# david-mathews-1994/deltarice

Hardware: AMD Instinct MI355X
Metric: encode+decode GB/s (int16 in) (higher is better)
Workload: dtype int16; 1 GPU; 1000000x7000 int16 Gaussian(sigma=10), m=8, 500 chunks of 2000x7000 per GPU, encode then decode, HBM resident; waveforms_per_gpu=1000000, wave_len=7000, rice_m=8, chunks_per_gpu=500, decode_impl=8

## Files before the change

### deltarice_amd/_lib.py

```python
from __future__ import annotations

import ctypes as C
import os

_HERE = os.path.dirname(os.path.abspath(__file__))
LIB_PATH = os.environ.get("DRX_LIB_PATH") or os.path.join(_HERE, "libdeltarice_hip.so")
PLUGIN_PATH = os.path.join(_HERE, "plugin", "libh5deltarice.so")

DRX_OK = 0
STATUS_NAMES = {0: "DRX_OK", 1: "DRX_ERR_ARG", 2: "DRX_ERR_DEVICE", 3: "DRX_ERR_CAPACITY",
                4: "DRX_ERR_CORRUPT", 5: "DRX_ERR_UNSUPPORTED", 6: "DRX_ERR_NOMEM"}
DRX_MAX_TAPS = 64

PATH_LANES_FUSED, PATH_LANES, PATH_BLOCKS, PATH_LONG, PATH_SIMPLE, PATH_IIR, PATH_IIR_FUSED = 1, 2, 4, 8, 16, 32, 64
PATH_SELECT = 128
PATH_GATHER = 256
PATH_STATS = 512
PATH_TRANSCODE = 1024
PATH_WINDOW = 2048
PATH_PULSES = 4096
PATH_WINDOWS = 8192
PATH_BINS = 16384
PATH_STACK = 32768
STACK_COUNT, STACK_SUM, STACK_SUMSQ = range(3)
STACK_COLS = 3
BIN_SUM, BIN_SUMSQ, BIN_MIN, BIN_MAX = range(4)
BIN_COLS = 4
STAT_MIN, STAT_ARGMIN, STAT_MAX, STAT_ARGMAX, STAT_SUM, STAT_SUMSQ, STAT_HEAD_SUM, STAT_HEAD_SUMSQ = range(8)
STAT_COLS = 8
PULSE_START, PULSE_WIDTH, PULSE_PEAK, PULSE_ARGPEAK, PULSE_SUM = range(5)
PULSE_COLS = 5
ENC_TWO_PASS, ENC_SEGMENTS, ENC_FUSED, ENC_PIECES, ENC_STREAM, ENC_STREAM_SEGS = 1, 2, 3, 4, 5, 6
DBG_BINS_LANES = 64
DBG_BINS_ALL_FALLBACK = 128
DBG_NO_LONG_PATHS = 256
DBG_LONG_NOT_BLOCKS = 512
DBG_TRANSCODE_LANES = 1024
DBG_NO_PARALLEL_WALKS = 2048
DBG_NO_PIECES = 4096
DBG_FORCE_SEGMENTS = 8192
DBG_TRANSCODE_ALL_FALLBACK = 16384
DBG_FORCE_PIECES = 32768
DBG_NO_WIDE_FUSED = 65536
DBG_RAGGED_ONE_LANES_LAUNCH = 131072
DBG_STREAM_THREE_WGS = 262144
DBG_FORCE_STREAM = 524288
DBG_REFILTER_SERIAL = 1048576
DBG_IIR_SEPARATE = 2097152
DBG_FORCE_STREAM_SEGS = 4194304
DBG_WALK_BY_SCAN = 8388608
DBG_WALK_BY_CHAINS = 16777216
DBG_GATHER_OTHER_COPY = 33554432
DBG_STATS_LANES = 67108864
DBG_STATS_ALL_FALLBACK = 134217728
DBG_PULSES_LANES = 268435456
DBG_PULSES_ALL_FALLBACK = 536870912
DBG_WINDOWS_LANES = 1073741824
DBG_WINDOWS_ALL_FALLBACK = 2147483648
STATS_FORM_LANES, STATS_FORM_BLOCKS, STATS_FORM_FALLBACK_ALL = 1, 2, 4
PULSES_FORM_LANES, PULSES_FORM_BLOCKS, PULSES_FORM_FALLBACK_ALL = 1, 2, 4
PULSES_STAGE_CAP = 8
WINDOWS_FORM_LANES, WINDOWS_FORM_BLOCKS, WINDOWS_FORM_FALLBACK_ALL = 1, 2, 4
BINS_FORM_LANES, BINS_FORM_BLOCKS, BINS_FORM_FALLBACK_ALL = 1, 2, 4
TRANSCODE_FORM_LANES, TRANSCODE_FORM_BLOCKS, TRANSCODE_FORM_FALLBACK_ALL = 1, 2, 4
TRANSCODE_FORM_REFILTER, TRANSCODE_FORM_REFILTER_SERIAL = 8, 16


class DrxOpts(C.Structure):
    _fields_ = [("rice_k", C.c_uint32), ("wave_len", C.c_int64), ("n_taps", C.c_uint32),
                ("taps", C.c_int32 * DRX_MAX_TAPS)]


class DeltaRiceError(RuntimeError):
    def __init__(self, status: int, msg: str = ""):
        self.status = status
        super().__init__(f"{STATUS_NAMES.get(status, status)}: {msg}")


_vp, _u64, _u32 = C.c_void_p, C.c_uint64, C.c_uint32
SIGNATURES = {
    "drx_version": (C.c_char_p, []),
    "drx_status_str": (C.c_char_p, [C.c_int]),
    "drx_device_count": (C.c_int, []),
    "drx_parse_cd_values": (C.c_int, [C.c_size_t, C.POINTER(C.c_uint), C.POINTER(DrxOpts)]),
    "drx_ctx_create": (C.c_int, [C.c_int, _vp, C.POINTER(_vp)]),
    "drx_ctx_destroy": (None, [_vp]),
    "drx_ctx_synchronize": (C.c_int, [_vp]),
    "drx_ctx_last_error": (C.c_char_p, [_vp]),
    "drx_ctx_stream": (_vp, [_vp]),
    "drx_ctx_device": (C.c_int, [_vp]),
    "drx_ctx_host_staging": (C.c_int, [_vp, C.c_size_t, C.POINTER(_vp)]),
    "drx_ctx_set_option": (C.c_int, [_vp, C.c_char_p, C.c_int64]),
    "drx_plan_create": (C.c_int, [_vp, _u64, C.POINTER(_u32), C.POINTER(_u32), _u32, C.POINTER(_vp)]),
    "drx_plan_create_uniform": (C.c_int, [_vp, _u64, _u32, _u32, _u32, C.POINTER(_vp)]),
    "drx_plan_set_filter": (C.c_int, [_vp, _u32, C.POINTER(C.c_int32)]),
    "drx_plan_destroy": (None, [_vp]),
    "drx_plan_n_chunks": (_u64, [_vp]),
    "drx_plan_total_samples": (_u64, [_vp]),
    "drx_plan_total_waves": (_u64, [_vp]),
    "drx_plan_max_encoded_words": (_u64, [_vp]),
    "drx_plan_wave_words": (_vp, [_vp]),
    "drx_plan_wave_word_off": (_vp, [_vp]),
    "drx_plan_last_decode_path": (C.c_uint32, [_vp]),
    "drx_plan_last_encode_path": (C.c_uint32, [_vp]),
    "drx_plan_last_stats_form": (C.c_uint32, [_vp]),
    "drx_plan_last_pulses_form": (C.c_uint32, [_vp]),
    "drx_plan_last_windows_form": (C.c_uint32, [_vp]),
    "drx_plan_last_windows_listed": (C.c_uint32, [_vp]),
    "drx_plan_last_bins_form": (C.c_uint32, [_vp]),
    "drx_plan_last_bins_listed": (C.c_uint32, [_vp]),
    "drx_plan_last_transcode_form": (C.c_uint32, [_vp]),
    "drx_plan_last_transcode_listed": (C.c_uint32, [_vp]),
    "drx_plan_last_pulses_listed": (C.c_uint32, [_vp]),
    "drx_plan_last_pulses_redone": (C.c_uint32, [_vp]),
    "drx_plan_read_wave_words": (C.c_int, [_vp, C.POINTER(_u32)]),
# ... 51 lines not shown
```

### deltarice_amd/csrc/drx_decode_kernels.hip

```cpp
#include <hip/hip_runtime.h>
#include <stdint.h>

#include <algorithm>
#include <type_traits>

#include "drx_internal.h"
#include "drx_device.h"
#include "drx_lane_stream.h"
#include "drx_walk.h"

namespace drx {

__global__ __launch_bounds__(64) void k_decode_simple(Geom G, const uint32_t *__restrict__ in,
                                                      const uint64_t *__restrict__ wave_off,
                                                      const uint32_t *__restrict__ wave_words, DevStatus *st,
                                                      int16_t *__restrict__ out, const uint32_t *__restrict__ only) {
    const uint64_t g = (uint64_t)blockIdx.x * 64u + threadIdx.x;
    if (g >= G.total_waves) return;
    if (only && !only[g]) return;
    const WaveRef r = locate(G, g);
    const uint32_t *s = in + wave_off[g] + 1;
    const uint32_t n = wave_words[g];
    int16_t *y = out + r.sample_off;
    int16_t hist[64];
// ... 512 lines not shown
    set_limits();
    auto commit_if_fits = [&]() __attribute__((always_inline)) {
        const uint32_t avail = (flw - ((~Q) >> 5)) & WMASK;
        if (pneed && avail <= (uint32_t)(RW - LW)) {
            store_piece(pv);
            pneed = false;
        }
    };
    auto group_refill = [&]() __attribute__((always_inline)) {
        if (__any((int32_t)(Q - Q_need) <= 0)) {
            commit_if_fits();
            wave_sync();
            sync_refill();
            set_limits();
        }
    };
    for (; t0 + T <= hi_min && t0 < steps; t0 += T) {
#pragma unroll 1
        for (int tg = 0; tg < T; tg += GS) {
            group_refill();
            decode_group(std::false_type{}, std::false_type{}, tg, 0u);
        }
        Q_end = (t0 + (uint32_t)T == hi_step) ? Q : Q_end;
        wave_sync();
        commit_if_fits();
        wave_sync();
        set_limits();
        if (!pneed) {
            const bool last = !(t0 + 2u * T <= hi_min && t0 + T < steps);
            const uint32_t avail = (flw - ((~Q) >> 5)) & WMASK;
            pneed = (flw < endw) && (!last || avail <= (uint32_t)(RW - LW));
            if (pneed) load_piece(pv);
        }
#pragma unroll
        for (int i = 0; i < PPS; ++i) {
            const int st = i * SPI + lane / PPS, p = lane % PPS;
            const uint4 v = orow16(st, p);
            store16(outg + wo_off[i] + t0, v);
        }
        wave_sync();
    }
    commit_if_fits();
    pneed = false;
    wave_sync();
    for (; t0 < steps; t0 += T) edge_round(t0);
    if (active && len && (((0u - Q_end) - 32u * s0 + 31u) >> 5) != n) atomicOr(&st->err, kErrCorrupt);
}

std::vector<uint2> decode_plan_ragged(Geom &G, const ChunkDesc *d) {
    const uint64_t n = G.n_chunks;
    uint32_t max_groups = 0, max_len = 0;
    for (uint64_t c = 0; c < n; ++c) {
        max_groups = std::max(max_groups, (d[c].n_waves + 63u) / 64u);
        max_len = std::max(max_len, d[c].wave_len);
    }
    G.max_groups = max_groups;
    G.max_wave_len64 = 64ull * max_len;
    std::vector<uint32_t> by_len(n);
    for (uint64_t c = 0; c < n; ++c) by_len[c] = (uint32_t)c;
    std::stable_sort(by_len.begin(), by_len.end(), [&](uint32_t a, uint32_t b) { return d[a].wave_len > d[b].wave_len; });
    std::vector<uint2> order;
    uint64_t n_long_groups = 0;
    for (uint32_t c : by_len)
        for (uint32_t j = 0; j < (d[c].n_waves + 63u) / 64u; ++j) {
            order.push_back(make_uint2(c, j));
            if (d[c].wave_len > kWalkShortLen) ++n_long_groups;
        }
    if (order.size() <= 0x7fffffffull) {
        G.rag_groups = (uint32_t)order.size();
        G.rag_groups_long = (uint32_t)n_long_groups;
    } else {
        order.clear();
    }
    return order;
}

enum class Dec { Simple, Blocks, Long, LanesFused, Lanes, LanesSplit };
enum class Walk { None, InLaunch, Parallel, Serial };
struct DecodeRoute {
    Dec dec;
    Walk walk;
    WalkRoute par;
    bool gen;
};

static DecodeRoute route_decode(const Geom &G, int impl, bool tables_ready, bool have_pw, bool have_blk, bool have_side) {
    DecodeRoute R{};
    R.gen = G.n_taps != 0;
    R.par = route_walk(G, tables_ready, have_pw);
    const bool simple = impl == 0 || (R.gen && !G.fast_taps);
    const bool want_fused = !tables_ready && impl == 8;
    const bool blocks = !simple && !(G.dbg & (DRX_DBG_NO_LONG_PATHS | DRX_DBG_LONG_NOT_BLOCKS)) && have_blk && blocks_batch(G) && (!R.gen || (G.iir_tab && G.iir_state));
    const bool longp = !simple && !blocks && !R.gen && !(G.dbg & DRX_DBG_NO_LONG_PATHS) && G.uniform && long_waveform_batch(G.total_waves, G.u_wave_len);
    const bool sparse = !G.uniform && (uint64_t)G.n_chunks * G.max_groups > 8ull * ((G.total_waves + 63u) / 64u) + 4096ull;
    R.dec = simple ? Dec::Simple : (blocks ? Dec::Blocks : (longp ? Dec::Long : Dec::Lanes));
    const bool parallel = R.par.chunk_wide || R.par.blocks;
    if (R.dec == Dec::Lanes && want_fused && !sparse && !parallel) R.dec = Dec::LanesFused;
    R.walk = tables_ready ? Walk::None : (R.dec == Dec::LanesFused ? Walk::InLaunch : (parallel ? Walk::Parallel : Walk::Serial));
    if (R.dec == Dec::Lanes && R.par.chunk_wide && R.par.blocks && have_side && G.rag_order && G.rag_groups_long &&
        G.rag_groups_long < G.rag_groups && !(G.dbg & DRX_DBG_RAGGED_ONE_LANES_LAUNCH)) R.dec = Dec::LanesSplit;
    return R;
}

hipError_t launch_decode(const StreamCall &c, int16_t *d_out, uint64_t *d_granules, int impl, void *d_blk, const SideStream *side,
                         uint32_t *path_out) {
    const Geom &G = *c.G;
    const hipStream_t s = c.s;
    uint32_t path_dummy = 0;
    uint32_t &path = path_out ? *path_out : path_dummy;
    path = 0;
    if (G.total_waves == 0) return hipSuccess;
    mark(c.ev, 0, s);
    const DecodeRoute R = route_decode(G, impl, c.tables_ready, c.d_pw != nullptr, d_blk != nullptr, side && side->s);
    const bool gen = R.gen;
    const unsigned nb_plain = blocks_for(G.total_waves, 64);

    auto launch_lanes = [&](const StreamCall &v, unsigned nb) {
        path |= DRX_PATH_LANES;
        if (gen)
            k_decode_lanes<false, true><<<nb, 64, 0, v.s>>>(*v.G, v.d_in, v.in_words, v.d_chunk_word_off, v.d_wave_off, v.d_wave_words, nullptr, nullptr, v.d_status, d_out);
        else
            k_decode_lanes<false><<<nb, 64, 0, v.s>>>(*v.G, v.d_in, v.in_words, v.d_chunk_word_off, v.d_wave_off, v.d_wave_words, nullptr, nullptr, v.d_status, d_out);
    };

    if (R.walk == Walk::InLaunch) {
        hipError_t e = hipMemsetAsync(d_granules, 0, (G.total_waves + 2) * sizeof(uint64_t), s);
        if (e != hipSuccess) return e;
    } else if (R.walk == Walk::Parallel) {
        const bool split = R.dec == Dec::LanesSplit;
        hipError_t e = walk_scratch_reset(G, c.d_pw, s);
        if (e != hipSuccess) return e;
        const bool forked = R.par.chunk_wide && R.par.blocks && side && side->s;
        hipStream_t spw = forked ? side->s : s;
        if (forked) {
            if ((e = hipEventRecord(side->fork, s)) != hipSuccess) return e;
            if ((e = hipStreamWaitEvent(side->s, side->fork, 0)) != hipSuccess) return e;
        }
        if (R.par.chunk_wide) launch_walk_chunk_wide(c.on(spw), R.par.by_chains);
        if (split) {
            Geom Gl = G;
            Gl.rag_groups = G.rag_groups_long;
            launch_lanes(c.view(Gl).on(spw), Gl.rag_groups);
        }
        if (forked && (e = hipEventRecord(side->join, side->s)) != hipSuccess) {
            (void)hipStreamSynchronize(side->s);
            return e;
        }
        if (R.par.blocks) launch_walk_blocks(c);
        if (split) {
            mark(c.ev, 1, s);
            Geom Gs = G;
            Gs.rag_order = G.rag_order + G.rag_groups_long;
            Gs.rag_groups = G.rag_groups - G.rag_groups_long;
            launch_lanes(c.view(Gs), Gs.rag_groups);
        }
        if (forked && (e = hipStreamWaitEvent(s, side->join, 0)) != hipSuccess) {
            (void)hipStreamSynchronize(side->s);
            return e;
        }
    } else if (R.walk == Walk::Serial) {
        launch_walk_serial(c);
    }
    if (R.dec != Dec::LanesSplit) mark(c.ev, 1, s);

    switch (R.dec) {
    case Dec::LanesFused: {
        uint32_t *ticket = reinterpret_cast<uint32_t *>(d_granules + G.total_waves);
        unsigned n_walk, groups;
        unsigned nb;
        if (G.uniform) {
            n_walk = (G.u_wave_len <= kWalkShortLen) ? (unsigned)G.n_chunks : blocks_for(G.n_chunks, kWalkChains);
            groups = (G.u_n_waves + 63u) / 64u;
            const uint32_t full = G.u_n_waves >> 6, rem = G.u_n_waves & 63u;
            nb = n_walk + (unsigned)(G.n_chunks * full) + (rem ? (unsigned)((G.n_chunks + 64u / rem - 1u) / (64u / rem)) : 0u);
        } else {
            n_walk = G.n_short + blocks_for(G.n_long, kWalkChains);
            groups = G.max_groups;
            nb = n_walk + (unsigned)(G.n_chunks * groups);
        }
        path |= DRX_PATH_LANES_FUSED;
        if (gen)
            k_decode_lanes<true, true><<<nb, 64, 0, s>>>(G, c.d_in, c.in_words, c.d_chunk_word_off, c.d_wave_off, c.d_wave_words, d_granules, ticket, c.d_status, d_out);
        else
            k_decode_lanes<true><<<nb, 64, 0, s>>>(G, c.d_in, c.in_words, c.d_chunk_word_off, c.d_wave_off, c.d_wave_words, d_granules, ticket, c.d_status, d_out);
        break;
    }
    case Dec::Blocks: {
        const uint32_t *fail = nullptr, *suspect = nullptr;
        bool fused = false;
        hipError_t e = launch_decode_blocks(c, d_blk, d_out, &fail, &suspect, gen, &fused);
        if (e != hipSuccess) return e;
        path |= DRX_PATH_BLOCKS | (gen ? (fused ? DRX_PATH_IIR_FUSED : DRX_PATH_IIR) : 0u);
        k_decode_long<<<(unsigned)G.total_waves, kLongThreads, 0, s>>>(G, c.d_in, c.d_wave_off, c.d_wave_words, c.d_status, d_out, fail, suspect, gen ? 1u : 0u);
        if (gen) {
            if (!fused && (e = launch_iir(G, G.iir_chunk_tile_base, G.iir_n_tiles, G.iir_tab, G.iir_state, fail, c.d_status, d_out, s)) != hipSuccess) return e;
            k_decode_simple<<<nb_plain, 64, 0, s>>>(G, c.d_in, c.d_wave_off, c.d_wave_words, c.d_status, d_out, fail);
        }
        break;
    }
    case Dec::Long:
        path |= DRX_PATH_LONG;
        k_decode_long<<<(unsigned)G.total_waves, kLongThreads, 0, s>>>(G, c.d_in, c.d_wave_off, c.d_wave_words, c.d_status, d_out, nullptr, nullptr, 0u);
// ... 18 lines not shown
```

### deltarice_amd/csrc/drx_internal.h

```cpp
#ifndef DRX_INTERNAL_H
#define DRX_INTERNAL_H

#include <hip/hip_runtime.h>
#include <stdint.h>

#include <type_traits>
#include <vector>

#include "../../include/deltarice_hip.h"

namespace drx {

struct ChunkDesc {
    uint64_t sample_off;
    uint64_t wave_base;
    uint32_t n_samples;
    uint32_t wave_len;
    uint32_t n_waves;
    uint32_t pad_;
};

struct Geom {
    const ChunkDesc *chunks;
    uint64_t n_chunks;
// ... 191 lines not shown
                              int64_t thr, bool neg, uint32_t min_width, uint32_t max_pulses, uint32_t *d_count, int64_t *d_out,
                              uint32_t *form_out);
uint64_t pulses_blocks_scratch_bytes(const Geom &G);
uint64_t pulses_blocks_staging_bytes(const Geom &G, uint32_t max_pulses);
hipError_t launch_pulses_blocks(const StreamCall &c, void *d_blk, void *d_ptab, void *d_pstage, const int64_t *d_thr, uint64_t thr_stride,
                                int64_t thr, bool neg, uint32_t min_width, uint32_t max_pulses, uint32_t *d_count, int64_t *d_out,
                                BlkFallbackList *list_out);
hipError_t launch_estimate_words(const Geom &G, const int16_t *d_in, unsigned long long *d_words16, hipStream_t s);
hipError_t launch_chunk_offsets(const Geom &G, const uint32_t *d_wave_words, uint32_t *d_wave_rel, uint64_t *d_chunk_words,
                                uint64_t *d_chunk_word_off, uint64_t out_cap, DevStatus *d_status, hipStream_t s);
struct TrcScratch {
    uint64_t *chunk_words;
    unsigned long long *est;
    uint32_t *words, *rel;
    uint64_t bytes;
};
inline TrcScratch trc_scratch_view(const Geom &G, void *base) {
    const uint64_t W = G.total_waves ? G.total_waves : 1, C = G.n_chunks + 1;
    TrcScratch t;
    t.chunk_words = (uint64_t *)base;
    t.est = (unsigned long long *)(t.chunk_words + C);
    t.words = (uint32_t *)(t.est + 16);
    t.rel = t.words + W;
    t.bytes = (C + 16) * sizeof(uint64_t) + 2 * W * sizeof(uint32_t);
    return t;
}
hipError_t launch_transcode(const StreamCall &c, uint32_t k2, const TrcScratch &t, const EncOut &out, void *d_blk, void *d_tb, uint32_t *form_out);
hipError_t launch_estimate_words_encoded(const StreamCall &c, unsigned long long *d_est, void *d_blk, void *d_tb, uint32_t *form_out);
uint64_t trc_blocks_scratch_bytes(const Geom &G);
hipError_t launch_trc_blocks_sizes(const StreamCall &c, void *d_blk, void *d_tb, uint32_t k2, const TrcScratch &t, uint32_t *d_out_wave_words,
                                   unsigned long long *d_est, BlkFallbackList *list_out);
hipError_t launch_trc_blocks_pack(const StreamCall &c, void *d_blk, void *d_tb, uint32_t k2, const TrcScratch &t, const EncOut &out);
struct RefilterTarget {
    uint32_t n_taps;
    const int32_t *taps;
};
hipError_t launch_refilter(const StreamCall &c, uint32_t k2, const RefilterTarget &T, const TrcScratch &t, const EncOut &out, uint32_t *form_out);
hipError_t launch_estimate_words_refiltered(const StreamCall &c, const RefilterTarget &T, unsigned long long *d_est, uint32_t *form_out);

hipError_t launch_encode_fused(const EncodeCall &c, int wide, uint64_t *d_scan);

constexpr uint32_t kEsRingWords = 2496;
constexpr uint64_t kEsMinUnits = 8192;
hipError_t launch_encode_stream(const EncodeCall &c, uint64_t *d_scan);

constexpr uint32_t kEsSegWaves = 4;
constexpr uint32_t kEsSegMinLen = 1024, kEsSegMaxLen = 7168;
struct EsSegShape { uint32_t seg_len, nseg, tpw; };
__host__ __device__ inline EsSegShape es_seg_shape(uint32_t L, uint32_t seg_target) {
    EsSegShape sh;
    uint32_t n = (L + seg_target - 1u) / seg_target;
    n = n ? n : 1u;
    const uint32_t dn = n / kEsSegWaves * kEsSegWaves, up = (n + kEsSegWaves - 1u) / kEsSegWaves * kEsSegWaves;
    n = up;
    if (dn && dn != up) {
        const uint64_t sd = (L + dn - 1u) / dn, su = (L + up - 1u) / up;
        const uint64_t pen_dn = sd > seg_target ? (sd - seg_target) * 55u : 0u, pen_up = su < seg_target ? (seg_target - su) * 40u : 0u;
        if (sd * 57u <= (uint64_t)seg_target * 67u && pen_dn < pen_up) n = dn;
    }
    sh.seg_len = (((L + n - 1u) / n) + 7u) & ~7u;
    sh.nseg = (L + sh.seg_len - 1u) / sh.seg_len;
    sh.tpw = (sh.nseg + kEsSegWaves - 1u) / kEsSegWaves;
    return sh;
}
inline bool stream_segs_admits(const Geom &G) { return G.uniform && (G.n_taps == 0 || G.enc_fast) && G.u_wave_len >= 64u &&
                                                       G.total_waves * es_seg_shape(G.u_wave_len, kEsSegMinLen).tpw < 0xffff0000ull; }
constexpr uint32_t kEsSegsFromLen = 20480;
inline uint64_t segs_scan_words(const Geom &G, uint32_t seg_target) { return 3 * G.total_waves * es_seg_shape(G.u_wave_len, seg_target).tpw + 192; }
hipError_t launch_encode_stream_segs(const EncodeCall &c, uint32_t seg_target, uint64_t *d_scan);

bool long_batch_admits(const Geom &G);
bool long_batch(const Geom &G);
uint64_t long_batch_units(const Geom &G);
std::vector<uint64_t> segments_plan_ragged(Geom &G, const ChunkDesc *host_chunks);
hipError_t launch_encode_long(const EncodeCall &c, uint32_t *d_wave_rel, uint64_t *d_chunk_words, uint32_t *d_seg_bits,
                              uint64_t *d_seg_pos);

struct SideStream {
    hipStream_t s;
    hipEvent_t fork, join;
};
hipError_t launch_decode(const StreamCall &c, int16_t *d_out, uint64_t *d_granules, int impl, void *d_blk, const SideStream *side,
                         uint32_t *path_out = nullptr);
bool blocks_batch(const Geom &G, double lane_us = 0.06, bool any_filter = false);
std::vector<uint32_t> blocks_plan_ragged(Geom &G, const ChunkDesc *host_chunks);
uint64_t blocks_scratch_bytes(const Geom &G);
uint64_t blocks_total_slots(const Geom &G);
hipError_t launch_decode_blocks(const StreamCall &c, void *d_blk, int16_t *d_out, const uint32_t **fail_out,
                                const uint32_t **suspect_out, bool resid, bool *fused_out);
constexpr uint32_t kBlkMaxClasses = 32;
struct BlkTables {
    uint32_t *fail, *suspect, *ends;
    uint64_t *state;
};
struct BlkClassLaunch {
    uint32_t *info;
    const uint32_t *list;
    uint32_t n_waves;
    int nt, sw;
    uint32_t spw, run_len;
    unsigned grid;
};
template <class F> inline void blk_dispatch(int nt, int sw, F f) {
    auto by_sw = [&](auto nt_tag) {
        switch (sw) {
            case 9: f(nt_tag, std::integral_constant<int, 9>{}); break;
            case 11: f(nt_tag, std::integral_constant<int, 11>{}); break;
            case 15: f(nt_tag, std::integral_constant<int, 15>{}); break;
            default: f(nt_tag, std::integral_constant<int, 19>{}); break;
        }
    };
    if (nt == 64) by_sw(std::integral_constant<int, 64>{});
    else if (nt == 128) by_sw(std::integral_constant<int, 128>{});
    else by_sw(std::integral_constant<int, 256>{});
}
hipError_t blocks_prepare(const Geom &G, uint64_t in_words, const uint32_t *d_wave_words, void *d_blk, hipStream_t s, BlkTables *T,
                          BlkClassLaunch *launches, uint32_t *n_launches);
uint32_t blocks_iir_tab_words();
void blocks_iir_tables(const uint32_t fast_nt[3], uint32_t t0neg, uint32_t *tab);
constexpr uint32_t kPcWaves = 8;
constexpr uint32_t kPcRunSamples = 7168;
constexpr uint32_t kPcMaxRun = 16;
constexpr uint32_t kPcSegSamples = 8192;
constexpr uint32_t kPcWholeLen = 10240;
constexpr uint32_t kPcMinLen = 64;
__host__ __device__ inline uint32_t pc_seg_samples(uint32_t k) {
    if (k <= 3u) return kPcSegSamples;
    const uint32_t s = (131072u / (2u * k + 9u)) & ~511u;
    return s < 512u ? 512u : s;
}
__host__ __device__ inline uint32_t pc_run_samples(uint32_t k) { return k <= 3u ? kPcRunSamples : pc_seg_samples(k) - 512u; }
__host__ __device__ inline uint32_t pc_whole_len(uint32_t k) { return k <= 3u ? kPcWholeLen : 65536u / (k + 4u); }
__host__ __device__ inline uint32_t pc_max_len(uint32_t k) { return pc_seg_samples(k) * kPcWaves; }
struct PieceShape {
    uint32_t run;
    uint32_t segs;
    uint32_t parts;
    uint32_t seg_len;
    uint32_t pieces;
    uint32_t wgs;
};
__host__ __device__ inline bool piece_packable(uint32_t L) { return L >= 8u && L < 512u && (L & 7u) == 0u; }
__host__ __device__ inline PieceShape piece_shape(uint32_t L, uint32_t W, uint32_t k, bool packed) {
    PieceShape s;
    s.parts = 1u;
    const uint32_t run_samples = pc_run_samples(k), seg_samples = pc_seg_samples(k), max_len = pc_max_len(k);
    if (packed) {
        const uint32_t bits = k <= 3u ? 9u : k + 6u;
        uint32_t by_samples = run_samples / L, by_words = 2000u / (1u + (bits * L + 31u) / 32u);
        by_samples = by_samples ? by_samples : 1u;
        by_words = by_words ? by_words : 1u;
        s.run = by_samples < by_words ? by_samples : by_words;
        s.segs = 1u;
        s.seg_len = L;
        s.pieces = (W + s.run - 1u) / s.run;
        s.wgs = (s.pieces + kPcWaves - 1u) / kPcWaves;
    } else if (L <= run_samples / 2u) {
        s.run = run_samples / L < kPcMaxRun ? run_samples / L : kPcMaxRun;
        s.segs = 1u;
        s.seg_len = L;
        s.pieces = (W + s.run - 1u) / s.run;
        s.wgs = (s.pieces + kPcWaves - 1u) / kPcWaves;
    } else if (L <= max_len) {
        const uint32_t need = L <= pc_whole_len(k) ? 1u : (L + seg_samples - 1u) / seg_samples;
        s.run = 1u;
        s.segs = 1u;
// ... 40 lines not shown
```

### include/deltarice_hip.h

```cpp
#ifndef DELTARICE_HIP_H
#define DELTARICE_HIP_H

#include <stddef.h>
#include <stdint.h>

#ifdef __cplusplus
extern "C" {
#endif

#define DRX_FILTER_ID 32025
#define DRX_MAX_TAPS 64

typedef struct drx_ctx drx_ctx;
typedef struct drx_plan drx_plan;

typedef enum {
    DRX_OK = 0,
    DRX_ERR_ARG = 1,
    DRX_ERR_DEVICE = 2,
    DRX_ERR_CAPACITY = 3,
    DRX_ERR_CORRUPT = 4,
    DRX_ERR_UNSUPPORTED = 5,
    DRX_ERR_NOMEM = 6
} drx_status;
// ... 131 lines not shown
#define DRX_PULSE_PEAK 2
#define DRX_PULSE_ARGPEAK 3
#define DRX_PULSE_SUM 4
#define DRX_PULSE_COLS 5
drx_status drx_find_pulses(drx_plan *plan, const uint32_t *d_in, uint64_t in_words, const uint64_t *d_chunk_word_off,
                           const int64_t *d_thr, uint64_t thr_stride, int64_t thr, int32_t polarity, uint32_t min_width,
                           uint32_t max_pulses, uint32_t *d_count, int64_t *d_out);
#define DRX_PULSES_FORM_LANES 1u
#define DRX_PULSES_FORM_BLOCKS 2u
#define DRX_PULSES_FORM_FALLBACK_ALL 4u
uint32_t drx_plan_last_pulses_form(const drx_plan *plan);
#define DRX_PULSES_STAGE_CAP 8u
uint32_t drx_plan_last_pulses_listed(const drx_plan *plan);
uint32_t drx_plan_last_pulses_redone(const drx_plan *plan);
drx_status drx_find_pulses_with_wave_words(drx_plan *plan, const uint32_t *d_in, uint64_t in_words,
                                           const uint64_t *d_chunk_word_off, const uint32_t *d_wave_words, const int64_t *d_thr,
                                           uint64_t thr_stride, int64_t thr, int32_t polarity, uint32_t min_width,
                                           uint32_t max_pulses, uint32_t *d_count, int64_t *d_out);

drx_status drx_transcode(drx_plan *plan, const uint32_t *d_in, uint64_t in_words, const uint64_t *d_chunk_word_off,
                         uint32_t new_rice_k, uint32_t *d_out, uint64_t out_cap_words, uint64_t *d_out_chunk_word_off,
                         uint32_t *d_out_wave_words);
drx_status drx_transcode_with_wave_words(drx_plan *plan, const uint32_t *d_in, uint64_t in_words, const uint64_t *d_chunk_word_off,
                                         const uint32_t *d_wave_words, uint32_t new_rice_k, uint32_t *d_out, uint64_t out_cap_words,
                                         uint64_t *d_out_chunk_word_off, uint32_t *d_out_wave_words);
drx_status drx_transcode_filter(drx_plan *plan, const uint32_t *d_in, uint64_t in_words, const uint64_t *d_chunk_word_off,
                                uint32_t new_rice_k, uint32_t new_n_taps, const int32_t *new_taps, uint32_t *d_out,
                                uint64_t out_cap_words, uint64_t *d_out_chunk_word_off, uint32_t *d_out_wave_words);
drx_status drx_transcode_filter_with_wave_words(drx_plan *plan, const uint32_t *d_in, uint64_t in_words,
                                                const uint64_t *d_chunk_word_off, const uint32_t *d_wave_words, uint32_t new_rice_k,
                                                uint32_t new_n_taps, const int32_t *new_taps, uint32_t *d_out, uint64_t out_cap_words,
                                                uint64_t *d_out_chunk_word_off, uint32_t *d_out_wave_words);
#define DRX_TRANSCODE_FORM_LANES 1u
#define DRX_TRANSCODE_FORM_BLOCKS 2u
#define DRX_TRANSCODE_FORM_FALLBACK_ALL 4u
#define DRX_TRANSCODE_FORM_REFILTER 8u
#define DRX_TRANSCODE_FORM_REFILTER_SERIAL 16u
uint32_t drx_plan_last_transcode_form(const drx_plan *plan);
uint32_t drx_plan_last_transcode_listed(const drx_plan *plan);
drx_status drx_estimate_words_encoded(drx_plan *plan, const uint32_t *d_in, uint64_t in_words, const uint64_t *d_chunk_word_off,
                                      const uint32_t *d_wave_words, uint64_t words_out[16]);
drx_status drx_estimate_words_encoded_filter(drx_plan *plan, const uint32_t *d_in, uint64_t in_words, const uint64_t *d_chunk_word_off,
                                             const uint32_t *d_wave_words, uint32_t new_n_taps, const int32_t *new_taps,
                                             uint64_t words_out[16]);

drx_status drx_estimate_words(drx_plan *plan, const int16_t *d_in, uint64_t words_out[16]);

drx_status drx_plan_finish(drx_plan *plan, uint64_t *total_words);

const uint32_t *drx_plan_wave_words(const drx_plan *plan);
const uint64_t *drx_plan_wave_word_off(const drx_plan *plan);
#define DRX_PATH_LANES_FUSED 1u
#define DRX_PATH_LANES 2u
#define DRX_PATH_BLOCKS 4u
#define DRX_PATH_LONG 8u
#define DRX_PATH_SIMPLE 16u
#define DRX_PATH_IIR 32u
#define DRX_PATH_IIR_FUSED 64u
#define DRX_PATH_SELECT 128u
#define DRX_PATH_GATHER 256u
#define DRX_PATH_STATS 512u
#define DRX_PATH_TRANSCODE 1024u
#define DRX_PATH_WINDOW 2048u
#define DRX_PATH_PULSES 4096u
#define DRX_PATH_WINDOWS 8192u
#define DRX_PATH_BINS 16384u
#define DRX_PATH_STACK 32768u
uint32_t drx_plan_last_decode_path(const drx_plan *plan);
#define DRX_ENC_TWO_PASS 1u
#define DRX_ENC_SEGMENTS 2u
#define DRX_ENC_FUSED 3u
#define DRX_ENC_PIECES 4u
#define DRX_ENC_STREAM 5u
#define DRX_ENC_STREAM_SEGS 6u
uint32_t drx_plan_last_encode_path(const drx_plan *plan);
drx_status drx_plan_read_wave_words(drx_plan *plan, uint32_t *host_out);

drx_status drx_filter_chunk_host(drx_ctx *ctx, int reverse, size_t cd_nelmts,
                                 const unsigned *cd_values, const void *in, size_t nbytes,
                                 void **out, size_t *out_bytes);

drx_status drx_plan_last_timings(drx_plan *plan, float ms[4]);

#define DRX_DBG_BINS_LANES 64u
#define DRX_DBG_BINS_ALL_FALLBACK 128u
#define DRX_DBG_NO_LONG_PATHS 256u
#define DRX_DBG_LONG_NOT_BLOCKS 512u
#define DRX_DBG_TRANSCODE_LANES 1024u
#define DRX_DBG_NO_PARALLEL_WALKS 2048u
#define DRX_DBG_NO_PIECES 4096u
#define DRX_DBG_FORCE_SEGMENTS 8192u
#define DRX_DBG_TRANSCODE_ALL_FALLBACK 16384u
#define DRX_DBG_FORCE_PIECES 32768u
#define DRX_DBG_NO_WIDE_FUSED 65536u
#define DRX_DBG_RAGGED_ONE_LANES_LAUNCH 131072u
#define DRX_DBG_STREAM_THREE_WGS 262144u
#define DRX_DBG_FORCE_STREAM 524288u
#define DRX_DBG_REFILTER_SERIAL 1048576u
#define DRX_DBG_IIR_SEPARATE 2097152u
#define DRX_DBG_FORCE_STREAM_SEGS 4194304u
#define DRX_DBG_WALK_BY_SCAN 8388608u
#define DRX_DBG_WALK_BY_CHAINS 16777216u
#define DRX_DBG_GATHER_OTHER_COPY 33554432u
#define DRX_DBG_STATS_LANES 67108864u
#define DRX_DBG_STATS_ALL_FALLBACK 134217728u
#define DRX_DBG_PULSES_LANES 268435456u
#define DRX_DBG_PULSES_ALL_FALLBACK 536870912u
#define DRX_DBG_WINDOWS_LANES 1073741824u
#define DRX_DBG_WINDOWS_ALL_FALLBACK 2147483648u
drx_status drx_ctx_set_option(drx_ctx *ctx, const char *key, int64_t value);

#ifdef __cplusplus
}
#endif
#endif
```

Baseline: 1557 GB/s.

## Add lane-per-wave decode kernel with smaller LDS footprint for eight waves per CU

Adds a new lanes decode kernel that shrinks the per-wavefront shared-memory ring and output staging so eight wavefronts fit per CU, decodes two Rice symbols per step in the steady state, and prefetches the next input piece into registers while the current round's output is written. It is routed in when the lanes path is chosen with impl 8 and the total work is deep enough relative to the longest wave, with debug flags to force or disable it. The kernel is considerably more complex, with edge rounds handled separately, and a smaller ring means more frequent refills.

```diff
diff --git a/deltarice_amd/_lib.py b/deltarice_amd/_lib.py
--- a/deltarice_amd/_lib.py
+++ b/deltarice_amd/_lib.py
@@ -31,6 +31,8 @@
 PULSE_START, PULSE_WIDTH, PULSE_PEAK, PULSE_ARGPEAK, PULSE_SUM = range(5)
 PULSE_COLS = 5
 ENC_TWO_PASS, ENC_SEGMENTS, ENC_FUSED, ENC_PIECES, ENC_STREAM, ENC_STREAM_SEGS = 1, 2, 3, 4, 5, 6
+DBG_LANES_EIGHT_PER_CU = 16
+DBG_LANES_SIX_PER_CU = 32
 DBG_BINS_LANES = 64
 DBG_BINS_ALL_FALLBACK = 128
 DBG_NO_LONG_PATHS = 256
diff --git a/deltarice_amd/csrc/drx_decode_kernels.hip b/deltarice_amd/csrc/drx_decode_kernels.hip
--- a/deltarice_amd/csrc/drx_decode_kernels.hip
+++ b/deltarice_amd/csrc/drx_decode_kernels.hip
@@ -618,6 +618,7 @@
     Walk walk;
     WalkRoute par;
     bool gen;
+    bool lanes8;
 };
 
 static DecodeRoute route_decode(const Geom &G, int impl, bool tables_ready, bool have_pw, bool have_blk, bool have_side) {
@@ -635,6 +636,11 @@
     R.walk = tables_ready ? Walk::None : (R.dec == Dec::LanesFused ? Walk::InLaunch : (parallel ? Walk::Parallel : Walk::Serial));
     if (R.dec == Dec::Lanes && R.par.chunk_wide && R.par.blocks && have_side && G.rag_order && G.rag_groups_long &&
         G.rag_groups_long < G.rag_groups && !(G.dbg & DRX_DBG_RAGGED_ONE_LANES_LAUNCH)) R.dec = Dec::LanesSplit;
+    constexpr uint64_t kLaneSlots = 98304;
+    const uint64_t longest = G.uniform ? G.u_wave_len : G.max_wave_len64 / 64u;
+    const bool deep = longest * kLaneSlots <= G.total_samples;
+    R.lanes8 = (R.dec == Dec::Lanes || R.dec == Dec::LanesSplit) && !R.gen && impl == 8 && !(G.dbg & DRX_DBG_LANES_SIX_PER_CU) &&
+               (deep || (G.dbg & DRX_DBG_LANES_EIGHT_PER_CU));
     return R;
 }
 
@@ -653,7 +659,9 @@
 
     auto launch_lanes = [&](const StreamCall &v, unsigned nb) {
         path |= DRX_PATH_LANES;
-        if (gen)
+        if (R.lanes8)
+            launch_decode_lanes8(v, nb, d_out);
+        else if (gen)
             k_decode_lanes<false, true><<<nb, 64, 0, v.s>>>(*v.G, v.d_in, v.in_words, v.d_chunk_word_off, v.d_wave_off, v.d_wave_words, nullptr, nullptr, v.d_status, d_out);
         else
             k_decode_lanes<false><<<nb, 64, 0, v.s>>>(*v.G, v.d_in, v.in_words, v.d_chunk_word_off, v.d_wave_off, v.d_wave_words, nullptr, nullptr, v.d_status, d_out);
diff --git a/deltarice_amd/csrc/drx_decode_lanes8.hip b/deltarice_amd/csrc/drx_decode_lanes8.hip
--- /dev/null
+++ b/deltarice_amd/csrc/drx_decode_lanes8.hip
@@ -0,0 +1,316 @@
+#include <hip/hip_runtime.h>
+#include <stdint.h>
+
+#include <type_traits>
+
+#include "drx_internal.h"
+#include "drx_device.h"
+
+namespace drx {
+
+__global__ __launch_bounds__(64, 1) void k_decode_lanes8(Geom G, const uint32_t *__restrict__ in, uint64_t in_words,
+                                                         const uint64_t *__restrict__ wave_off,
+                                                         const uint32_t *__restrict__ wave_words, DevStatus *st,
+                                                         int16_t *__restrict__ out) {
+    constexpr int RW = 64;
+    constexpr int LW = 32;
+    constexpr int T = 64;
+    constexpr int GS = 16;
+    constexpr int LOG_RW = 6;
+    constexpr int OSW = GS / 2 + 4;
+    constexpr int PPS = T / 8;
+    constexpr int SPI = 64 / PPS;
+    constexpr int NV = LW / 4;
+    constexpr uint32_t WMASK = (1u << 27) - 1u;
+    constexpr uint32_t NEED_AT = GS + 2;
+    static_assert(T % GS == 0 && RW - LW >= GS + 2, "round length / ring slack");
+    static_assert(GS == 16 && PPS == 8, "a group is two 16-byte pieces of every row");
+    __shared__ uint32_t ring_all[(RW + 2) * 64];
+    uint32_t *const ring = ring_all + 64;
+    __shared__ __attribute__((aligned(16))) uint32_t obuf[64 * OSW];
+    uint64_t *tab_off = reinterpret_cast<uint64_t *>(obuf);
+    uint32_t *tab_lo = obuf + 128, *tab_hi = obuf + 192;
+    static_assert(64 * OSW >= 256, "tables fit in obuf");
+    static_assert(sizeof(ring_all) + sizeof(obuf) <= 20480, "eight wavefronts per CU");
+
+    const int lane = lane_id();
+    const uint32_t k = G.k;
+    typedef uint32_t u32x4v __attribute__((ext_vector_type(4)));
+    typedef u32x4v __attribute__((address_space(1))) g_uint4;
+    typedef int16_t __attribute__((address_space(1))) g_i16;
+    g_i16 *const outg = (g_i16 *)out;
+    uint64_t g;
+    bool active;
+    uint32_t len = 0, n = 0;
+    uint64_t S = 1, ooff = 0;
+    const uint32_t wave_idx = blockIdx.x;
+    if (!G.uniform && G.rag_order) {
+        if (wave_idx >= G.rag_groups) return;
+        const uint2 e = G.rag_order[wave_idx];
+        const ChunkDesc d = G.chunks[e.x];
+        const uint32_t idx = e.y * 64u + (uint32_t)lane;
+        active = idx < d.n_waves;
+        g = d.wave_base + idx;
+        if (active) {
+            len = (idx + 1 == d.n_waves) ? (d.n_samples - idx * d.wave_len) : d.wave_len;
+            ooff = d.sample_off + (uint64_t)idx * d.wave_len;
+            S = wave_off[g] + 1u;
+            n = wave_words[g];
+        }
+    } else {
+        g = (uint64_t)wave_idx * 64u + lane;
+        active = g < G.total_waves;
+        if (active) {
+            const WaveRef r = locate(G, g);
+            len = r.len;
+            ooff = r.sample_off;
+            S = wave_off[g] + 1u;
+            n = wave_words[g];
+        }
+    }
+    const uint32_t phi = active ? (uint32_t)((((uintptr_t)out >> 1) + ooff) & (uint64_t)(T - 1)) : 0u;
+    const uint32_t steps = wave_max_u32(len + phi);
+    const uint32_t lo_max = wave_max_u32(phi);
+    const uint32_t hi_min = ~wave_max_u32(~(phi + len));
+    uint64_t wo_off[PPS];
+    uint32_t wo_lo[PPS], wo_hi[PPS];
+    tab_off[lane] = ooff - phi;
+    tab_lo[lane] = phi;
+    tab_hi[lane] = phi + len;
+    wave_sync();
+#pragma unroll
+    for (int i = 0; i < PPS; ++i) {
+        const int st_i = i * SPI + lane / PPS, p = lane % PPS;
+        wo_off[i] = tab_off[st_i] + 8u * (uint32_t)p;
+        wo_lo[i] = tab_lo[st_i];
+        wo_hi[i] = tab_hi[st_i];
+    }
+    wave_sync();
+
+    const uint64_t A = (S & ~(uint64_t)(RW - 1)) - (uint64_t)RW;
+    const uint32_t s0 = (uint32_t)(S - A);
+    const uint32_t endw = s0 + n;
+    uint32_t flw = s0 & ~(uint32_t)(LW - 1);
+    const bool in_vec_ok = ((uintptr_t)in & 15u) == 0;
+    uint32_t *myring = ring + lane;
+    typedef uint16_t __attribute__((may_alias)) u16a;
+    u16a *myout = reinterpret_cast<u16a *>(obuf + lane * OSW);
+
+    uint4 v[PPS] = {};
+    const int my_group = (lane % PPS) >> 1;
+    const uint32_t *my_rows = obuf + (lane / PPS) * OSW + 4 * (lane & 1);
+    auto read_back = [&](int tg) __attribute__((always_inline)) {
+        if (tg / GS == my_group) {
+#pragma unroll
+            for (int i = 0; i < PPS; ++i) v[i] = *reinterpret_cast<const uint4 *>(my_rows + i * SPI * OSW);
+        }
+    };
+
+    auto load_piece = [&](uint4 (&pv)[NV]) {
+        const uint64_t a = A + flw;
+        if (in_vec_ok && a + (uint32_t)LW <= in_words) {
+#pragma unroll
+            for (int j = 0; j < NV; ++j) pv[j] = *reinterpret_cast<const uint4 *>(in + a + 4 * j);
+        } else {
+#pragma unroll
+            for (int j = 0; j < NV; ++j) {
+                pv[j].x = (a + 4 * j + 0 < in_words) ? in[a + 4 * j + 0] : 0u;
+                pv[j].y = (a + 4 * j + 1 < in_words) ? in[a + 4 * j + 1] : 0u;
+                pv[j].z = (a + 4 * j + 2 < in_words) ? in[a + 4 * j + 2] : 0u;
+                pv[j].w = (a + 4 * j + 3 < in_words) ? in[a + 4 * j + 3] : 0u;
+            }
+        }
+    };
+    auto store_piece = [&](const uint4 (&pv)[NV]) {
+        const uint32_t r0 = (uint32_t)RW - (flw & (uint32_t)(RW - 1));
+        uint32_t *dst = myring + r0 * 64u;
+#pragma unroll
+        for (int j = 0; j < NV; ++j) {
+            dst[-(4 * j + 0) * 64] = pv[j].x; dst[-(4 * j + 1) * 64] = pv[j].y;
+            dst[-(4 * j + 2) * 64] = pv[j].z; dst[-(4 * j + 3) * 64] = pv[j].w;
+        }
+        if (r0 == (uint32_t)RW) {
+            myring[0] = pv[0].x;
+            myring[-64] = pv[0].y;
+        }
+        flw += (uint32_t)LW;
+    };
+
+    uint32_t Q = 0u - 32u * s0;
+    uint32_t Q_need;
+    auto set_limits = [&]() __attribute__((always_inline)) {
+        const bool more = flw < endw;
+        Q_need = more ? ~(32u * (flw - NEED_AT + 1u)) : Q - 0x7fffffffu;
+    };
+    auto sync_refill = [&]() __attribute__((always_inline)) {
+        for (;;) {
+            const uint32_t avail = (flw - ((~Q) >> 5)) & WMASK;
+            const bool more = flw < endw;
+            if (!__any(more && avail < NEED_AT)) break;
+            if (more && avail <= (uint32_t)(RW - LW)) {
+                uint4 pv[NV];
+                load_piece(pv);
+                store_piece(pv);
+            }
+            wave_sync();
+        }
+    };
+
+    {
+        uint4 pv[NV];
+        for (int i = 0; i < RW / LW; ++i) {
+            if (__ballot(flw < endw && flw + (uint32_t)LW <= s0 + (uint32_t)RW) == 0) break;
+            if (flw < endw && flw + (uint32_t)LW <= s0 + (uint32_t)RW) {
+                load_piece(pv);
+                store_piece(pv);
+            }
+        }
+        wave_sync();
+    }
+    int32_t acc = 0;
+
+    const uint32_t hi_step = phi + len;
+    uint32_t Q_end = 0;
+    auto decode_group = [&](auto first_tag, auto edge_tag, int tg, uint32_t tcur) __attribute__((always_inline)) {
+        constexpr bool FIRST = decltype(first_tag)::value;
+        constexpr bool EDGE = decltype(edge_tag)::value;
+        if (!FIRST) {
+#pragma unroll
+            for (int u = 0; u < GS; u += 2) {
+                const uint32_t row = __builtin_amdgcn_ubfe(Q, 5u, (uint32_t)LOG_RW);
+                const uint32_t *wp = myring + row * 64u;
+                const uint32_t lo = wp[0], hi = wp[64], lo2 = wp[-64];
+                const uint32_t winA = __builtin_amdgcn_alignbit(hi, lo, Q);
+                const uint32_t winB = __builtin_amdgcn_alignbit(lo, lo2, Q);
+                const uint32_t q1 = ffbh(winA);
+                const uint32_t kk1 = (winA < (1u << 24)) ? 16u : k;
+                const uint32_t nu1 = ~(q1 + kk1);
+                const uint32_t win2 = __builtin_amdgcn_alignbit(winA, winB, nu1);
+                const uint32_t q2 = ffbh(win2);
+                const uint32_t kk2 = (win2 < (1u << 24)) ? 16u : k;
+                const uint32_t nu2 = ~(q2 + kk2);
+                if constexpr (EDGE) {
+                    Q_end = (tcur + (uint32_t)u + 1u == hi_step) ? Q + nu1 : Q_end;
+                    Q_end = (tcur + (uint32_t)u + 2u == hi_step) ? Q + nu1 + nu2 : Q_end;
+                }
+                asm("v_add3_u32 %0, %1, %2, %3" : "=v"(Q) : "v"(Q), "v"(nu1), "v"(nu2));
+                const uint32_t z1 = (q1 << kk1) + __builtin_amdgcn_ubfe(winA, nu1, kk1);
+                const uint32_t z2 = (q2 << kk2) + __builtin_amdgcn_ubfe(win2, nu2, kk2);
+                acc += (int32_t)(z1 >> 1) ^ -(int32_t)(z1 & 1u);
+                const uint32_t a1 = (uint32_t)acc;
+                acc += (int32_t)(z2 >> 1) ^ -(int32_t)(z2 & 1u);
+                *reinterpret_cast<uint32_t *>(myout + u) = __builtin_amdgcn_perm((uint32_t)acc, a1, 0x05040100u);
+            }
+            return;
+        }
+#pragma unroll
+        for (int u = 0; u < GS; ++u) {
+            const uint32_t row = __builtin_amdgcn_ubfe(Q, 5u, (uint32_t)LOG_RW);
+            const uint32_t *wp = myring + row * 64u;
+            const uint32_t lo = wp[0], hi = wp[64];
+            const uint32_t win = __builtin_amdgcn_alignbit(hi, lo, Q);
+            const uint32_t q = ffbh(win);
+            const bool esc = win < (1u << 24);
+            const uint32_t kk = esc ? 16u : k;
+            const uint32_t used = q + kk + 1u;
+            const uint32_t rem = __builtin_amdgcn_ubfe(win, 32u - used, kk);
+            const uint32_t z = (q << kk) + rem;
+            const int32_t d = (int32_t)(z >> 1) ^ -(int32_t)(z & 1u);
+            const bool act = (uint32_t)(tg + u) >= phi;
+            acc = act ? acc + d : acc;
+            Q = act ? Q - used : Q;
+            if constexpr (EDGE) Q_end = (tcur + (uint32_t)u + 1u == hi_step) ? Q : Q_end;
+            myout[u] = (uint16_t)acc;
+        }
+    };
+
+    auto emit_masked = [&](g_i16 *dst, uint32_t lo, uint32_t hi, uint32_t t0, const uint4 &x) __attribute__((always_inline)) {
+        const int p = lane % PPS;
+        const uint32_t tpos = t0 + 8u * (uint32_t)p;
+        if (tpos + 8u > lo && tpos < hi) {
+            if (tpos >= lo && tpos + 8u <= hi) {
+                *(g_uint4 *)dst = (u32x4v){x.x, x.y, x.z, x.w};
+            } else {
+                const uint32_t w[4] = {x.x, x.y, x.z, x.w};
+#pragma unroll
+                for (int j = 0; j < 8; ++j)
+                    if (tpos + (uint32_t)j >= lo && tpos + (uint32_t)j < hi)
+                        dst[j] = (int16_t)(w[j >> 1] >> (16 * (j & 1)));
+            }
+        }
+    };
+    auto edge_round = [&](auto first_tag, uint32_t t0) __attribute__((always_inline)) {
+#pragma unroll 1
+        for (int tg = 0; tg < T; tg += GS) {
+            sync_refill();
+            decode_group(first_tag, std::true_type{}, tg, t0 + (uint32_t)tg);
+            wave_sync();
+            read_back(tg);
+            wave_sync();
+        }
+        if (t0 >= lo_max && t0 + T <= hi_min) {
+#pragma unroll
+            for (int i = 0; i < PPS; ++i) *(g_uint4 *)(outg + wo_off[i] + t0) = (u32x4v){v[i].x, v[i].y, v[i].z, v[i].w};
+        } else {
+#pragma unroll
+            for (int i = 0; i < PPS; ++i) emit_masked(outg + wo_off[i] + t0, wo_lo[i], wo_hi[i], t0, v[i]);
+        }
+    };
+
+    if (steps > 0) edge_round(std::true_type{}, 0u);
+    uint32_t t0 = T;
+    for (; t0 < steps && !(t0 >= lo_max && t0 + T <= hi_min); t0 += T) edge_round(std::false_type{}, t0);
+
+    uint4 pv[NV];
+    bool pneed = false;
+    set_limits();
+    auto commit_if_fits = [&]() __attribute__((always_inline)) {
+        const uint32_t avail = (flw - ((~Q) >> 5)) & WMASK;
+        if (pneed && avail <= (uint32_t)(RW - LW)) {
+            store_piece(pv);
+            pneed = false;
+        }
+    };
+    auto group_refill = [&]() __attribute__((always_inline)) {
+        if (__any((int32_t)(Q - Q_need) <= 0)) {
+            commit_if_fits();
+            wave_sync();
+            sync_refill();
+            set_limits();
+        }
+    };
+    for (; t0 + T <= hi_min && t0 < steps; t0 += T) {
+#pragma unroll 1
+        for (int tg = 0; tg < T; tg += GS) {
+            group_refill();
+            decode_group(std::false_type{}, std::false_type{}, tg, 0u);
+            wave_sync();
+            read_back(tg);
+            wave_sync();
+        }
+        Q_end = (t0 + (uint32_t)T == hi_step) ? Q : Q_end;
+        commit_if_fits();
+        wave_sync();
+        set_limits();
+        if (!pneed) {
+            const bool last = !(t0 + 2u * T <= hi_min && t0 + T < steps);
+            const uint32_t avail = (flw - ((~Q) >> 5)) & WMASK;
+            pneed = (flw < endw) && (!last || avail <= (uint32_t)(RW - LW));
+            if (pneed) load_piece(pv);
+        }
+#pragma unroll
+        for (int i = 0; i < PPS; ++i)
+            *(g_uint4 *)(outg + wo_off[i] + t0) = (u32x4v){v[i].x, v[i].y, v[i].z, v[i].w};
+    }
+    commit_if_fits();
+    pneed = false;
+    wave_sync();
+    for (; t0 < steps; t0 += T) edge_round(std::false_type{}, t0);
+    if (active && len && (((0u - Q_end) - 32u * s0 + 31u) >> 5) != n) atomicOr(&st->err, kErrCorrupt);
+}
+
+void launch_decode_lanes8(const StreamCall &c, unsigned nb, int16_t *d_out) {
+    k_decode_lanes8<<<nb, 64, 0, c.s>>>(*c.G, c.d_in, c.in_words, c.d_wave_off, c.d_wave_words, c.d_status, d_out);
+}
+
+}
diff --git a/deltarice_amd/csrc/drx_internal.h b/deltarice_amd/csrc/drx_internal.h
--- a/deltarice_amd/csrc/drx_internal.h
+++ b/deltarice_amd/csrc/drx_internal.h
@@ -297,6 +297,7 @@
 };
 hipError_t launch_decode(const StreamCall &c, int16_t *d_out, uint64_t *d_granules, int impl, void *d_blk, const SideStream *side,
                          uint32_t *path_out = nullptr);
+void launch_decode_lanes8(const StreamCall &c, unsigned nb, int16_t *d_out);
 bool blocks_batch(const Geom &G, double lane_us = 0.06, bool any_filter = false);
 std::vector<uint32_t> blocks_plan_ragged(Geom &G, const ChunkDesc *host_chunks);
 uint64_t blocks_scratch_bytes(const Geom &G);
diff --git a/include/deltarice_hip.h b/include/deltarice_hip.h
--- a/include/deltarice_hip.h
+++ b/include/deltarice_hip.h
@@ -237,6 +237,8 @@
 
 drx_status drx_plan_last_timings(drx_plan *plan, float ms[4]);
 
+#define DRX_DBG_LANES_EIGHT_PER_CU 16u
+#define DRX_DBG_LANES_SIX_PER_CU 32u
 #define DRX_DBG_BINS_LANES 64u
 #define DRX_DBG_BINS_ALL_FALLBACK 128u
 #define DRX_DBG_NO_LONG_PATHS 256u
```

New measurement: 1583 GB/s, median of 6. About the same (+1.7%).
